# ranok92/gym-ballenv

Measured on AMD Instinct MI355X. Metric: env-steps/sec (whole node), batch=65536 envs, window=10; achieved HBM GB/s, higher is better.
Workload: dtype int16x2+f64

## Files before the change

gym-ballenv_amd/csrc/ballenv.hip:

```cpp
#include <type_traits>
#include <hip/hip_runtime.h>

#include <math.h>
#include <algorithm>
#include <mutex>
#include <new>
#include <stdint.h>
#include <stdio.h>
#include <stdlib.h>
#include <string.h>

#include "ballenv.h"
#include "internal.h"
#include "philox.h"
#include "policy_core.h"

namespace {

constexpr uint32_t PURPOSE_STEP_OBS = 1, PURPOSE_ACTION = 2, PURPOSE_RESET = 3, PURPOSE_SAMPLE = 4;
constexpr int REJECT_LIMIT = 4096;
constexpr int CS = 16;
constexpr int CD = 8;
constexpr int HW_MAX = 63;

enum Mode { MODE_STEP = 0, MODE_RESET = 1, MODE_OBSERVE = 2 };

struct Tables {
  int32_t goal[BE_MAX_GOALS];
  int32_t action[BE_MAX_ACTIONS];
  int32_t speed[BE_MAX_DYNAMIC];
  int32_t strip_obs_x, strip_obs_y, strip_goal_x, strip_goal_y, strip_agent_x, strip_agent_y;
  int32_t radius_obstacle, radius_agent;
  uint8_t n_other[BE_MAX_GOALS];
  uint8_t other[BE_MAX_GOALS][BE_MAX_GOALS];
  uint8_t hw[HW_MAX + 1];
};

constexpr int SPAN_N = 72;
struct TablesX {
  Tables t;
  uint64_t span[SPAN_N];
};
static_assert(sizeof(Tables) % 16 == 0 && sizeof(TablesX) % 16 == 0, "16-byte table staging");
__host__ __device__ constexpr bool span_fits(int W, int R) {
  return W >= 2 && R >= 0 && W - 1 + 2 * R <= 63 && 2 * R + 2 * (W - 1) - 1 <= SPAN_N;
}

struct KParams {
  int32_t* agent; int32_t* goal; double* prev_dist; double* total_dist;
  double* ep_return; int32_t* ep_len; uint32_t* episode; int32_t* static_obs;
  int32_t* dyn_obs; uint8_t* dyn_goal; uint8_t* obs; float* obs_f32;
  double* reward; uint8_t* done; const uint8_t* actions; const Tables* tables;
  int32_t n, window, ns, nd, R, speed_x, speed_y, screen_w;
  int32_t screen_h, goal_change, certainty, time_limit, num_actions, autoreset, gid0, dbg;
  double threshold_goal, time_penalty, static_penalty, dynamic_penalty, min_spawn_dist;
  double inv_g1;
  unsigned long long seed;
  int* status;
  const int16_t* deltas; const int16_t* tape; const uint8_t* mask; const int16_t* reset_tape;
  uint8_t* truncated; uint8_t* terminal_obs; double* final_return; int32_t* final_len;
  double* stats;
  int32_t reset_tape_len;
  int32_t min_spawn_d2;
  uint32_t amx, amy;
  int32_t num_goals;
  int32_t prev_read;
  int32_t steps;
  int32_t pol_bytes, pol_actions;
  const uint8_t* pol_img;
  const uint8_t* obs_in;
  uint8_t* obs_last;
  uint8_t* act_out; float* logp_out; float* value_out;
  unsigned long long pol_seed;
  uint32_t* pool;
};

constexpr uint32_t POOL_VALID = 1u, POOL_REJ = 2u;
constexpr int PB_ROWS = 0, PB_AGENT = 3, PB_GOAL = 4, PB_PREV = 6, PB_TOTAL = 8, PB_OBS = 10;
__host__ __device__ constexpr int pool_body_words(int ns, int nd) { return (PB_OBS + ns + nd + 3) & ~3; }
__host__ __device__ constexpr int64_t pool_bytes_per_env(int ns, int nd) { return 2 * (8 + 4ll * pool_body_words(ns, nd)); }
static_assert(pool_body_words(13, 5) == 28, "the fixed-shape kernels' 112-byte entry body");
__device__ __forceinline__ uint32_t pool_body(uint32_t n, uint32_t x, int nbw) { return 16u * n + x * (4u * (uint32_t)nbw); }
template <class T>
__device__ __forceinline__ T pool_ld(const uint32_t* pool, uint32_t off, uint32_t imm = 0) {
  return *reinterpret_cast<const T*>(reinterpret_cast<const char*>(pool) + (size_t)off + imm);
}
template <class T>
__device__ __forceinline__ void pool_st(uint32_t* pool, uint32_t off, T v, uint32_t imm = 0) {
  *reinterpret_cast<T*>(reinterpret_cast<char*>(pool) + (size_t)off + imm) = v;
}
#ifndef BE_POOL_MODE
#define BE_POOL_MODE 1
#endif
__device__ __forceinline__ uint32_t u4w(const uint4& v, int k) { return k == 0 ? v.x : k == 1 ? v.y : k == 2 ? v.z : v.w; }
__device__ __forceinline__ double u2d(uint32_t lo, uint32_t hi) {
  return __longlong_as_double((long long)(((unsigned long long)hi << 32) | lo));
}
constexpr int64_t POOL_MAX_ENVS = 1ll << 22;

#define BE_DIAG_UNIT_STEP 1
#include "diag.h"

__device__ __forceinline__ int px(int32_t p) { return (int)(int16_t)(p & 0xFFFF); }
__device__ __forceinline__ int py(int32_t p) { return p >> 16; }
__device__ __forceinline__ int32_t pk(int x, int y) {
  return (int32_t)(((uint32_t)x & 0xFFFFu) | ((uint32_t)y << 16));
}
__device__ __forceinline__ uint32_t d2u(int dx, int dy) {
  uint32_t ax = (uint32_t)abs(dx), ay = (uint32_t)abs(dy);
  return ax * ax + ay * ay;
}
__device__ __forceinline__ int d2i(int dx, int dy) { return dx * dx + dy * dy; }
template <class T>
__device__ __forceinline__ T ld_s(const T* base, uint32_t idx) {
  return *reinterpret_cast<const T*>(reinterpret_cast<const char*>(base) + (size_t)(idx * (uint32_t)sizeof(T)));
}
#ifndef BE_S2_CT
#define BE_S2_CT 256
#endif
constexpr int S2_CT = BE_S2_CT;
constexpr int ST_PLAIN = 0, ST_WT = 1;
template <class T>
__device__ __forceinline__ void st_wt(T* p, T v) {
  __hip_atomic_store(p, v, __ATOMIC_RELAXED, __HIP_MEMORY_SCOPE_AGENT);
}
template <class T>
__device__ __forceinline__ T& ld_s_ptr(T* base, uint32_t idx) {
  return *reinterpret_cast<T*>(reinterpret_cast<char*>(base) + (size_t)(idx * (uint32_t)sizeof(T)));
}
template <class T>
__device__ __forceinline__ void st_ws(T* base, uint32_t idx, T v) {
  st_wt(&ld_s_ptr(base, idx), v);
}
__device__ __forceinline__ int isqrt_small(int n) {
  int s = (int)__builtin_amdgcn_sqrtf((float)n);
  if (s * s > n) --s;
  if ((s + 1) * (s + 1) <= n) ++s;
  return s;
}
__device__ __forceinline__ int floordiv(int a, int b) { return a >= 0 ? a / b : -((-a + b - 1) / b); }

typedef short v2s __attribute__((ext_vector_type(2)));

__device__ __forceinline__ uint32_t pick_word(const u4& b, int w) {
  return w == 0 ? b.x : (w == 1 ? b.y : (w == 2 ? b.z : b.w));
}
__device__ __forceinline__ uint32_t pick_field(const u4& b, int j) {
  constexpr uint32_t M = 0xFFFFFFu;
  return j == 0 ? (b.x & M)
       : j == 1 ? (__builtin_amdgcn_alignbit(b.y, b.x, 24) & M)
       : j == 2 ? (__builtin_amdgcn_alignbit(b.z, b.y, 16) & M)
       : j == 3 ? (b.z >> 8) : (b.w & M);
}
__device__ __forceinline__ int map_range(uint32_t r, int lo, int hi) {
  return lo + (int)__umulhi(r, (uint32_t)(hi - lo));
}

struct ResetDraws {
  const int16_t* tape; int32_t len; int32_t n; int32_t env; int32_t cursor;
  uint32_t gid; uint32_t episode; unsigned long long seed;
  int* status;
  __device__ int draw(int lo, int hi) {
    int k = cursor++;
    if (tape) {
      if (k >= len) { atomicOr(status, BE_STATUS_RESET_TAPE_EXHAUSTED); return lo; }
      return tape[(int64_t)k * n + env];
    }
    u4 b = philox(gid, episode, 0u, tag(PURPOSE_RESET, (uint32_t)k >> 2), seed);
    return map_range(pick_word(b, k & 3), lo, hi);
  }
};

__device__ __forceinline__ double sqrt_int(double x) {
  const double y = __builtin_amdgcn_rsq(x);
  double g = x * y, h = y * 0.5;
  const double r = __builtin_fma(-h, g, 0.5);
  g = __builtin_fma(g, r, g);
  h = __builtin_fma(h, r, h);
  double d = __builtin_fma(-g, g, x);
  g = __builtin_fma(d, h, g);
  d = __builtin_fma(-g, g, x);
  g = __builtin_fma(d, h, g);
  return x == 0.0 ? x : g;
}

__device__ __forceinline__ double calc_dist(int x1, int y1, int x2, int y2) {
  double dx = (double)(x1 - x2), dy = (double)(y1 - y2);
  return sqrt_int(dx * dx + dy * dy);
}
__device__ __forceinline__ double calc_dist_lib(int x1, int y1, int x2, int y2) {
  double dx = (double)(x1 - x2), dy = (double)(y1 - y2);
  return sqrt(dx * dx + dy * dy);
}

struct Win {
  int x0, y0;
  int sx, sy;
  int w;
  int kr;
  int R, R2;
  __device__ Win(const KParams& p, int ax, int ay) {
    w = p.window; const int h = w / 2;
    sx = p.speed_x; sy = p.speed_y;
    x0 = ax - sx * h; y0 = ay - sy * h;
    kr = w > 1 ? w - 1 : 1;
    R = p.R; R2 = R * R;
  }
  __device__ __forceinline__ bool near(int ox, int oy, int& f, int& e) const {
    f = ox - x0; e = oy - y0;
    const int cx = min(max(f, 0), sx * (w - 1));
    const int cy = min(max(e, 0), sy * (kr - 1));
    return d2u(f - cx, e - cy) <= (uint32_t)R2;
  }
};

__device__ __forceinline__ int quadrant(int ax, int ay, int gx, int gy) {
  const int dx = gx - ax, dy = gy - ay;
  if (dx >= 0 && dy >= 0) return 1;
  if (dx < 0 && dy >= 0) return 0;
  if (dx < 0 && dy < 0) return 3;
  return 2;
}

__device__ __forceinline__ uint32_t lds_bytes(const void* lo, const void* hi) {
  return (uint32_t)(uintptr_t)hi - (uint32_t)(uintptr_t)lo;
}

template <int BLOCK>
struct NearList {
  uint32_t* base; int cnt;
  __device__ __forceinline__ void push(int f, int e) {
    base[cnt * BLOCK] = (uint32_t)(f & 0xFFFF) | ((uint32_t)e << 16);
    ++cnt;
  }
  __device__ __forceinline__ void push_if(bool c, int f, int e) {
    if (c) push(f, e);
  }
  __device__ __forceinline__ void get(int n, int& f, int& e) const {
    const uint32_t v = base[n * BLOCK];
    f = (int)(int16_t)(v & 0xFFFF); e = (int)v >> 16;
  }
};

template <int WT> struct Geo {
  static constexpr int K = WT > 1 ? WT - 1 : 1;
  static constexpr int NW = (WT * WT + 31) / 32 + 1;
  static constexpr int F = 4 + WT * WT;
};

template <int WT, int BLOCK, bool HWT = false>
__device__ __forceinline__ void raster_rows(const NearList<BLOCK>& nl, const Win& g, uint32_t (&rows)[Geo<WT>::K],
                                            const uint8_t* hwt = nullptr) {
  constexpr int K = Geo<WT>::K;
#pragma unroll
  for (int k = 0; k < K; ++k) rows[k] = 0u;
  if constexpr (HWT) {
    for (int n = 0; n < nl.cnt; ++n) {
      int f, e;
      nl.get(n, f, e);
      f += WT / 2; e += WT / 2;
#pragma unroll
      for (int k = 0; k < K; ++k) {
        const int ady = abs(e - k);
        const int hw = hwt[min(ady, HW_MAX)];
        const int lo = max(f - hw, 0), hi = min(f + hw, WT - 1);
        rows[k] |= (ady <= g.R && lo <= hi) ? (2u << hi) - (1u << lo) : 0u;
      }
    }
    return;
// ... 1141 lines not shown
        const int nr = min(RCAP, nres - r0);
        if (r0 > 0) {
          if (valid && lead && s_slot_of[el] >= r0 && s_slot_of[el] < r0 + RCAP) {
            const int s = s_slot_of[el] - r0;
            s_reset_el[s] = (int16_t)el; s_reset_ep[s] = episode + 1u;
          }
          __syncthreads();
        }
        if (tid < nr) {
          const int e_l = s_reset_el[tid];
          const int ir = blk0 + e_l;
          const uint32_t ep = s_reset_ep[tid];
          const uint32_t g_id = (uint32_t)p.gid0 + (uint32_t)ir;
          const int W = p.screen_w, H = p.screen_h;
          const u4 b0 = philox(g_id, ep, 0u, tag(PURPOSE_RESET, 0), p.seed);
          const int rgx = map_range(b0.x, W - t.strip_goal_x, W), rgy = map_range(b0.y, H - t.strip_goal_y, H);
          int rax = map_range(b0.z, 0, t.strip_agent_x), ray = map_range(b0.w, 0, t.strip_agent_y);
          const double dist = calc_dist(rgx, rgy, rax, ray);
          for (int r = 0; calc_dist(rgx, rgy, rax, ray) < p.min_spawn_dist; ++r) {
            if (r >= REJECT_LIMIT - 1) { atomicOr(p.status, BE_STATUS_REJECTION_LIMIT); break; }
            const u4 b = philox(g_id, ep, 0u, tag(PURPOSE_RESET, 1 + r), p.seed);
            rax = map_range(b.x, 0, t.strip_agent_x); ray = map_range(b.y, 0, t.strip_agent_y);
          }
          p.agent[ir] = pk(rax, ray);
          p.goal[ir] = pk(rgx, rgy);
          p.prev_dist[ir] = dist;
          p.total_dist[ir] = calc_dist(rax, ray, rgx, rgy);
          p.ep_return[ir] = 0.0;
          p.ep_len[ir] = 0;
          p.episode[ir] = ep;
          s_reset_agent[tid] = pk(rax, ray);
          s_reset_goal[tid] = pk(rgx, rgy);
#pragma unroll
          for (int k = 0; k < KR; ++k) s_rows[tid][k] = 0u;
        }
        __syncthreads();
        DIAG(12);
        const int per = Ns + Nd;
        const int R = t.radius_obstacle + t.radius_agent;
        const int rx = R, ry2 = t.radius_obstacle + 2 * t.radius_agent;
        for (int it = tid; it < nr * per; it += BLOCK_THREADS) {
          const int s = it / per, k = it - s * per;
          const int ir = blk0 + s_reset_el[s];
          const uint32_t ep = s_reset_ep[s];
          const uint32_t g_id = (uint32_t)p.gid0 + (uint32_t)ir;
          const int rax = px(s_reset_agent[s]), ray = py(s_reset_agent[s]);
          const int rgx = px(s_reset_goal[s]), rgy = py(s_reset_goal[s]);
          const int W = p.screen_w, H = p.screen_h;
          int ox, oy;
          if (k < Ns) {
            for (int at = 0;; ++at) {
              const u4 b = philox(g_id, ep, 0u, tag(PURPOSE_RESET, (1u << 22) | ((uint32_t)k << 12) | (uint32_t)at), p.seed);
              ox = map_range(b.x, t.strip_obs_x, W - t.strip_obs_x);
              oy = map_range(b.y, t.strip_obs_y, H - t.strip_obs_y);
              const bool ra = abs(ox - rax) < rx && 2 * abs(oy - ray) < ry2;
              const bool rg = abs(ox - rgx) < rx && 2 * abs(oy - rgy) < ry2;
              if (!ra && !rg) break;
              if (at >= REJECT_LIMIT - 1) { atomicOr(p.status, BE_STATUS_REJECTION_LIMIT); break; }
            }
            (p.static_obs + (size_t)k * N)[ir] = pk(ox, oy);
          } else {
            const int kd = k - Ns;
            const u4 b = philox(g_id, ep, 0u, tag(PURPOSE_RESET, (2u << 22) | ((uint32_t)kd << 12)), p.seed);
            ox = map_range(b.x, t.strip_obs_x, W - t.strip_obs_x);
            oy = map_range(b.y, t.strip_obs_y, H - t.strip_obs_y);
            (p.dyn_obs + (size_t)kd * N)[ir] = pk(ox, oy);
            (p.dyn_goal + (size_t)kd * N)[ir] = (uint8_t)kd;
          }
          const Win g(p, rax, ray);
          int f, e;
          if (g.near(ox, oy, f, e)) raster_one_lds<WT>(s_rows[s], g, f, e);
        }
        __syncthreads();
        DIAG(13);
        if (tid < nr) {
          uint32_t rows[Geo<WT>::K], fl[Geo<WT>::NW];
#pragma unroll
          for (int k = 0; k < Geo<WT>::K; ++k) rows[k] = s_rows[tid][k];
          flatten<WT>(rows, fl);
          const int e_l = s_reset_el[tid];
          const int32_t ag = s_reset_agent[tid], go = s_reset_goal[tid];
          stage_full_row<WT>(stage + e_l * F, fl, quadrant(px(ag), py(ag), px(go), py(go)));
        }
        __syncthreads();
        DIAG(14);
      }
    }
    DIAG(5);
    const int nvalid = min(EPB, N - blk0);
    copy_out<BLOCK_THREADS>(stage, F, nvalid, (int64_t)blk0, p.obs, p.obs_f32);
  } else {
    if (valid && lead) {
      const int F = 4 + p.window * p.window;
      const Win g(p, ax, ay);
      write_row_generic<BLOCK_THREADS>(nl, g, quadrant(ax, ay, gx, gy), p.obs ? p.obs + (int64_t)i * F : nullptr,
                                       p.obs_f32 ? p.obs_f32 + (int64_t)i * F : nullptr);
    }
    if (MODE == MODE_STEP && (tid & 63) == 0) s_ws[tid >> 6] = ws;
    __syncthreads();
  }

  DIAG(6);
  if (MODE == MODE_STEP && p.stats && tid == 0) {
    WaveStats b = s_ws[0];
#pragma unroll
    for (int w = 1; w < BLOCK_THREADS / 64; ++w) {
      const WaveStats& o = s_ws[w];
      b.n += o.n; b.s1 += o.s1; b.s2 += o.s2; b.sl += o.sl; b.mn = fmin(b.mn, o.mn); b.mx = fmax(b.mx, o.mx);
    }
    if (b.n > 0.0) {
      double* slot = p.stats + (size_t)blockIdx.x * 8;
      slot[0] += b.n; slot[1] += b.s1; slot[2] += b.s2; slot[3] += b.sl;
      slot[4] = fmin(slot[4], b.mn); slot[5] = fmax(slot[5], b.mx);
    }
  }
}

__device__ __forceinline__ uint32_t mul24_byte(uint32_t x, uint32_t k, int sel) {
  uint32_t r;
  switch (sel) {
    case 0: asm("v_mul_u32_u24_sdwa %0, %1, %2 dst_sel:DWORD dst_unused:UNUSED_PAD src0_sel:BYTE_0 src1_sel:DWORD" : "=v"(r) : "v"(x), "v"(k)); break;
    case 1: asm("v_mul_u32_u24_sdwa %0, %1, %2 dst_sel:DWORD dst_unused:UNUSED_PAD src0_sel:BYTE_1 src1_sel:DWORD" : "=v"(r) : "v"(x), "v"(k)); break;
    case 2: asm("v_mul_u32_u24_sdwa %0, %1, %2 dst_sel:DWORD dst_unused:UNUSED_PAD src0_sel:BYTE_2 src1_sel:DWORD" : "=v"(r) : "v"(x), "v"(k)); break;
    default: asm("v_mul_u32_u24_sdwa %0, %1, %2 dst_sel:DWORD dst_unused:UNUSED_PAD src0_sel:BYTE_3 src1_sel:DWORD" : "=v"(r) : "v"(x), "v"(k)); break;
  }
  return r;
}
__device__ __forceinline__ uint32_t pair_or(uint32_t x) {
  return x | (uint32_t)__builtin_amdgcn_update_dpp(0, (int)x, 0xB1, 0xF, 0xF, false);
}

template <int WT, int NSC, int NDC, bool POOL = false>
__global__ __launch_bounds__(S2_CT, 2) void step2_kernel(KParams p) {
  constexpr int CT = S2_CT;
  constexpr int L = 2, EPW = 64 / L, EPB = CT / L, NWAVE = CT / 64;
  constexpr int SS = (NSC + L - 1) / L, SD = (NDC + L - 1) / L;
  constexpr int KR = Geo<WT>::K, F = Geo<WT>::F, NW = Geo<WT>::NW;
  constexpr int NQ = F / 8, HQ = (NQ + 1) / 2;
  static_assert(WT == 10 && F == 104 && NW == 5, "the half-row word split below is laid out for W = 10");
  static_assert(NDC <= 5, "one Philox block of 24-bit fields");
  static_assert(16 * KR >= (64 / (NSC + NDC)) * (KR + 4), "wave reset scratch");
  extern __shared__ __align__(16) uint8_t smem[];
  __shared__ __align__(16) TablesX t_wave[NWAVE];
  __shared__ uint32_t s_rows[NWAVE][16 * KR];
  constexpr int TW = (int)(sizeof(TablesX) / 16);

  DIAG(0);
  if (DBG(DBG_EXIT_ENTRY)) return;
  const int N = p.n, tid = (int)threadIdx.x, w = tid >> 6, lane = tid & 63, h = lane & 1;
  const int blk0 = (int)blockIdx.x * EPB, i = blk0 + (tid >> 1), e0 = blk0 + w * EPW;
  uint8_t* stage_blk = smem + (size_t)(SS + SD + 1) * CT * 4;
  const bool valid = i < N;
  const uint32_t ic = (uint32_t)min(i, N - 1), gid = (uint32_t)p.gid0 + (uint32_t)i;
  NearList<CT> nl{reinterpret_cast<uint32_t*>(smem) + tid, 0};
  Tables& t = t_wave[w].t;
  const uint64_t* span = t_wave[w].span;
  uint8_t* stage = stage_blk + (size_t)w * EPW * F;
  constexpr int TB = 64;
  const int tt0 = lane;

  constexpr int TL = (TW + TB - 1) / TB;
  uint4 tword[TL];
#pragma unroll
  for (int j = 0; j < TL; ++j)
    tword[j] = ld_s(reinterpret_cast<const uint4*>(p.tables), (uint32_t)min(tt0 + j * TB, TW - 1));
  const uint32_t episode = ld_s(p.episode, ic);
  const int len0 = ld_s(p.ep_len, ic);
  const int32_t agent0 = ld_s(p.agent, ic), goal0 = ld_s(p.goal, ic);
  int32_t dp[SD], so[SS];
  int dgi[SD];
#pragma unroll
  for (int j = 0; j < SD; ++j) {
    const uint32_t e = (uint32_t)min(L * j + h, NDC - 1) * (uint32_t)N + ic;
    dp[j] = ld_s(p.dyn_obs, e);
    dgi[j] = ld_s(p.dyn_goal, e);
  }
#pragma unroll
  for (int j = 0; j < SS; ++j) so[j] = ld_s(p.static_obs, (uint32_t)min(L * j + h, NSC - 1) * (uint32_t)N + ic);
  const double old_dist = p.prev_read ? ld_s(p.prev_dist, ic) : calc_dist(px(goal0), py(goal0), px(agent0), py(agent0));
  const double total = ld_s(p.total_dist, ic);
  double ret = ld_s(p.ep_return, ic);
  const int a = ld_s(p.actions, ic);
  double* const slot = p.stats ? p.stats + (size_t)(e0 / 32) * 8 : nullptr;
  double2 sp0 = make_double2(0.0, 0.0), sp1 = sp0, sp2 = sp0;
  if (slot && lane == 0 && e0 < N) {
    sp0 = reinterpret_cast<const double2*>(slot)[0];
    sp1 = reinterpret_cast<const double2*>(slot)[1];
    sp2 = reinterpret_cast<const double2*>(slot)[2];
  }
#pragma unroll
  for (int j = 0; j < TL; ++j) reinterpret_cast<uint4*>(&t_wave[w])[min(tt0 + j * TB, TW - 1)] = tword[j];
  __builtin_amdgcn_fence(__ATOMIC_RELEASE, "wavefront");
  __builtin_amdgcn_wave_barrier();
  __builtin_amdgcn_fence(__ATOMIC_ACQUIRE, "wavefront");
  DIAG(1);
  if (DBG(DBG_EXIT_BARRIER)) return;
  if (DBG(DBG_WAIT_LOADS)) {
    __builtin_amdgcn_s_waitcnt(0);
    DIAG(15);
  }

  int counter = (int)((double)len0 * p.inv_g1);
  counter = len0 - counter * (p.goal_change + 1);
  if (counter < 0) counter += p.goal_change + 1;
  if (counter > p.goal_change) counter -= p.goal_change + 1;
  const bool change = counter >= p.goal_change;
  const u4 b0 = DBG(DBG_NO_PHILOX) ? u4{gid, episode, (uint32_t)len0, gid ^ episode}
                                   : philox(gid, episode, (uint32_t)len0, tag(PURPOSE_STEP_OBS, 0u), p.seed);
  DIAG(7);
  uint32_t st_flags = 0u;
  int ngs[SD];
  int32_t dnew[SD];
#pragma unroll
  for (int j = 0; j < SD; ++j) {
    const int k = L * j + h;
    const bool real = k < NDC;
    int ox = px(dp[j]), oy = py(dp[j]);
    const uint32_t f = h ? pick_field(b0, min(L * j + 1, 4)) : pick_field(b0, L * j);
    uint32_t fl = 0u;
    ngs[j] = dyn_move_fixed(p, t, ox, oy, dgi[j], t.speed[min(k, NDC - 1)], change, f, fl);
    st_flags |= real ? fl : 0u;
    dnew[j] = pk(ox, oy);
  }
  DIAG(11);
  st_flags |= a >= p.num_actions ? (uint32_t)BE_STATUS_BAD_ACTION : 0u;
  const uint32_t sh = 2u * (uint32_t)(a < p.num_actions ? a : 0);
  int ax = min(max(px(agent0) + (int)((p.amx >> sh) & 3u) - 1, 0), p.screen_w);
  int ay = min(max(py(agent0) + (int)((p.amy >> sh) & 3u) - 1, 0), p.screen_h);
  int gx = px(goal0), gy = py(goal0);
  const Win g0(p, 0, 0);
  const uint32_t R2 = (uint32_t)g0.R2;
  const NearBox nb0(g0);
  typedef unsigned short v2u __attribute__((ext_vector_type(2)));
  const v2s boxo = {(short)(WT / 2 + g0.R), (short)(WT / 2 + g0.R)};
  const v2u boxw = {(unsigned short)nb0.bw, (unsigned short)nb0.bh};
  const v2s agv = __builtin_bit_cast(v2s, pk(ax, ay));
  const double dist = calc_dist(gx, gy, ax, ay);
  const double rbase = (0.0 - p.time_penalty) + (old_dist - dist) / total;
  DIAG(8);
  bool hs = false, hd = false;
  uint32_t* nlp = nl.base;
  auto obstacle_pk = [&](int32_t opk, bool real, bool& hit) {
    const v2s d = __builtin_elementwise_sub_sat(__builtin_bit_cast(v2s, opk), agv);
    hit |= real & ((uint32_t)dot2_sq(d) <= R2);
    const v2u b = __builtin_bit_cast(v2u, __builtin_elementwise_add_sat(d, boxo));
    const v2u over = __builtin_elementwise_sub_sat(b, boxw);
    *nlp = __builtin_bit_cast(uint32_t, d);
    const uint32_t in = __builtin_elementwise_sub_sat(1u, __builtin_bit_cast(uint32_t, over) | (real ? 0u : 1u));
    nlp += CT * in;
  };
#pragma unroll
  for (int j = 0; j < SD; ++j) obstacle_pk(dnew[j], L * j + h < NDC, hd);
#pragma unroll
  for (int j = 0; j < SS; ++j) obstacle_pk(so[j], L * j + h < NSC, hs);
  nl.cnt = (int)(lds_bytes(nl.base, nlp) / (CT * 4u));
  hs = pair_or((uint32_t)hs) != 0u;
  hd = pair_or((uint32_t)hd) != 0u;
  DIAG(10);

  double reward = rbase;
  if (hs) reward -= p.static_penalty;
  else if (hd) reward -= p.dynamic_penalty;
  ret += reward;
  const int len = len0 + 1;
  const bool env_done = (dist < p.threshold_goal) || hs || hd;
  const bool trunc = p.time_limit > 0 && len >= p.time_limit;
  const bool done = env_done || trunc;
  const bool do_reset = valid && done && p.autoreset;
  const bool ptry = POOL && do_reset && p.pool != nullptr;
  uint2 q_tv = make_uint2(0u, 0u);
  uint4 qb[7];
#if BE_POOL_MODE == 1 || BE_POOL_MODE == 6
  if constexpr (POOL)
#if BE_POOL_MODE == 6
  if (__ballot(ptry))
#endif
  if (ptry) {
    const uint32_t x = ((episode + 1u) & 1u) * (uint32_t)N + (uint32_t)i;
    q_tv = pool_ld<uint2>(p.pool, x * 8u);
    const uint32_t bo = pool_body((uint32_t)N, x, 28);
#pragma unroll
    for (int j = 0; j < 7; ++j) qb[j] = pool_ld<uint4>(p.pool, bo, 16u * j);
    __builtin_amdgcn_s_waitcnt(0);
  }
#ifdef BE_DIAG_STAMPS
  if (__ballot(ptry)) DIAG(9);
#endif
#endif
  if (valid) {
    const uint32_t iu = (uint32_t)i;
    st_ws(p.reward, iu, reward);
    st_ws(p.ep_return, iu, ret);
    st_ws(p.agent, iu, pk(ax, ay));
    st_ws(p.ep_len, iu, len);
    if (p.done) st_ws(p.done, iu, (uint8_t)done);
    if (p.truncated) st_ws(p.truncated, iu, (uint8_t)(trunc && !env_done));
    st_ws(p.prev_dist, iu, dist);
    if (done) {
      if (p.final_return) st_ws(p.final_return, iu, ret);
      if (p.final_len) st_ws(p.final_len, iu, len);
    }
#pragma unroll
    for (int j = 0; j < SD; ++j) {
      const int k = L * j + h;
      if (k < NDC) {
        st_wt(&ld_s_ptr(p.dyn_obs, (uint32_t)k * (uint32_t)N + (uint32_t)i), dnew[j]);
        if (change) st_wt(&ld_s_ptr(p.dyn_goal, (uint32_t)k * (uint32_t)N + (uint32_t)i), (uint8_t)ngs[j]);
      }
    }
  }
  DIAG(2);
  if (__ballot(st_flags != 0u)) {
    uint32_t f = st_flags;
#pragma unroll
    for (int o = 32; o > 0; o >>= 1) f |= (uint32_t)__shfl_xor((int)f, o);
    if (lane == 0) atomicOr(p.status, (int)f);
  }
  if (DBG(DBG_EXIT_PHYSICS)) return;

  uint32_t xrows[KR];
#pragma unroll
  for (int k = 0; k < KR; ++k) xrows[k] = 0u;
  if (do_reset && p.terminal_obs) {
    uint32_t rows[KR], flat[NW];
    raster_rows_span<WT, CT>(nl, p.R, rows, span);
#pragma unroll
    for (int k = 0; k < KR; ++k) rows[k] = pair_or(rows[k]);
    flatten<WT>(rows, flat);
    if (!h) write_row_global<WT>(p.terminal_obs + (int64_t)i * F, flat, quadrant(ax, ay, gx, gy));
  }
  bool hit = false;
#if BE_POOL_MODE == 5
  const unsigned long long m0 = DBG(DBG_NO_RESET) ? 0ull : __ballot(do_reset && h == 0);
  if (m0) {
  if (POOL) {
    if (ptry) {
      const uint32_t x = ((episode + 1u) & 1u) * (uint32_t)N + (uint32_t)i;
      q_tv = pool_ld<uint2>(p.pool, x * 8u);
      const uint32_t bo = pool_body((uint32_t)N, x, 28);
#pragma unroll
      for (int j = 0; j < 7; ++j) qb[j] = pool_ld<uint4>(p.pool, bo, 16u * j);
    }
#else
  if (__ballot(ptry)) {
#endif
    hit = ptry && q_tv.x == episode + 1u && (q_tv.y & POOL_VALID) != 0u;
    if (hit) {
      auto qw = [&](int k) -> uint32_t { return u4w(qb[k >> 2], k & 3); };
      const uint32_t iu = (uint32_t)i;
      const int32_t ag = (int32_t)qw(PB_AGENT), go = (int32_t)qw(PB_GOAL);
      st_ws(p.ep_return, iu, 0.0);
      st_ws(p.ep_len, iu, 0);
      st_ws(p.agent, iu, ag);
      st_ws(p.prev_dist, iu, u2d(qw(PB_PREV), qw(PB_PREV + 1)));
      st_ws(p.goal, iu, go);
      st_ws(p.total_dist, iu, u2d(qw(PB_TOTAL), qw(PB_TOTAL + 1)));
      st_ws(p.episode, iu, episode + 1u);
#pragma unroll
      for (int j = 0; j < SD; ++j) {
        const int k = L * j + h;
        const uint32_t o = h ? qw(PB_OBS + NSC + min(L * j + 1, NDC - 1)) : qw(PB_OBS + NSC + L * j);
        if (k < NDC) {
          st_ws(p.dyn_obs, (uint32_t)k * (uint32_t)N + iu, (int32_t)o);
          st_ws(p.dyn_goal, (uint32_t)k * (uint32_t)N + iu, (uint8_t)k);
        }
      }
#pragma unroll
      for (int j = 0; j < SS; ++j) {
        const int k = L * j + h;
        const uint32_t o = h ? qw(PB_OBS + min(L * j + 1, NSC - 1)) : qw(PB_OBS + L * j);
        if (k < NSC) st_ws(p.static_obs, (uint32_t)k * (uint32_t)N + iu, (int32_t)o);
      }
      ax = px(ag); ay = py(ag); gx = px(go); gy = py(go);
#pragma unroll
      for (int k = 0; k < KR; ++k) xrows[k] = (qw(PB_ROWS + k / 3) >> (10 * (k % 3))) & 0x3FFu;
      nl.cnt = 0;
    }
    if (__ballot(hit && (q_tv.y & POOL_REJ)) && lane == 0) atomicOr(p.status, BE_STATUS_REJECTION_LIMIT);
  }
  const unsigned long long m = DBG(DBG_NO_RESET) ? 0ull : __ballot(do_reset && !hit && h == 0);
  if (m) {
    auto osink = [&](int, int k, int il, int32_t o) {
      if (k < NSC) {
        st_ws(p.static_obs, (uint32_t)k * (uint32_t)N + (uint32_t)il, o);
      } else {
        st_ws(p.dyn_obs, (uint32_t)(k - NSC) * (uint32_t)N + (uint32_t)il, o);
        st_ws(p.dyn_goal, (uint32_t)(k - NSC) * (uint32_t)N + (uint32_t)il, (uint8_t)(k - NSC));
      }
    };
    auto esink = [&](int, int32_t ag, int32_t go, int32_t a0) {
      double prev;
      const double td = reset_dists(ag, go, a0, prev);
      const uint32_t iu = (uint32_t)i;
      st_ws(p.ep_return, iu, 0.0);
      st_ws(p.ep_len, iu, 0);
      st_ws(p.agent, iu, ag);
      st_ws(p.prev_dist, iu, prev);
      st_ws(p.goal, iu, go);
      st_ws(p.total_dist, iu, td);
      st_ws(p.episode, iu, episode + 1u);
    };
    if (!(m & (m - 1)))
      wave_resets<WT, NSC, NDC, 1, decltype(osink)&, decltype(esink)&, L>(p, t, m, i, gid, episode, ax, ay, gx, gy,
                                                                        nl.cnt, xrows, &s_rows[w][0], osink, esink, span);
    else
      wave_resets<WT, NSC, NDC, 64, decltype(osink)&, decltype(esink)&, L>(p, t, m, i, gid, episode, ax, ay, gx, gy,
                                                                         nl.cnt, xrows, &s_rows[w][0], osink, esink, span);
  }
#if BE_POOL_MODE == 5
  }
#endif
  DIAG(3);
  if (DBG(DBG_NO_OBS)) return;
  if (DBG(DBG_NO_RASTER)) nl.cnt = 0;

  {
    uint32_t rows[KR];
    raster_rows_span<WT, CT>(nl, p.R, rows, span, xrows);
    const uint32_t P0 = pair_or(rows[0] | (rows[1] << 10) | (rows[2] << 20));
    const uint32_t P1 = pair_or(rows[3] | (rows[4] << 10) | (rows[5] << 20));
    const uint32_t P2 = pair_or(rows[6] | (rows[7] << 10) | (rows[8] << 20));
    const uint32_t vlo = h ? ((P1 >> 6) & 0xFFFFF0u) | (P2 << 24) : ((P0 << 4) & 0x3FF0u) | (P0 << 14);
    const uint32_t vhi = h ? P2 >> 8 : (P0 >> 18) | (P1 << 12);
    const unsigned long long c = (((unsigned long long)vhi << 32) | vlo) >> (6 * h);
    const uint32_t clo = (uint32_t)c, chi = (uint32_t)(c >> 32);
    const uint32_t ne0 = clo & 0x0F0F0F0Fu, no0 = (clo >> 4) & 0x0F0F0F0Fu;
    const uint32_t ne1 = chi & 0x0F0F0F0Fu, no1 = (chi >> 4) & 0x0F0F0F0Fu;
    const uint32_t kx = 0x00204081u;
    auto word = [&](int jj) -> uint32_t {
      const int b = jj >> 1;
      const uint32_t src = (jj & 1) ? (b < 4 ? no0 : no1) : (b < 4 ? ne0 : ne1);
      return mul24_byte(src, kx, b & 3) & 0x01010101u;
    };
    const uint32_t sx = (uint32_t)(gx - ax) >> 31, sy = (uint32_t)(gy - ay) >> 31;
    const uint32_t onehot = 1u << ((sy << 4) | ((sx ^ sy ^ 1u) << 3));
    uint2* dst = reinterpret_cast<uint2*>(stage + (tid & 62) / 2 * F) + HQ * h;
#pragma unroll
    for (int q = 0; q < HQ; ++q) {
      const uint32_t w0 = q == 0 ? (h ? word(0) : onehot) : word(2 * q);
      if (q < NQ - HQ || !h) dst[q] = make_uint2(w0, word(2 * q + 1));
    }
  }
  DIAG(4);
  __builtin_amdgcn_fence(__ATOMIC_RELEASE, "wavefront");
  __builtin_amdgcn_wave_barrier();
  __builtin_amdgcn_fence(__ATOMIC_ACQUIRE, "wavefront");
  DIAG(5);
  if (!DBG(DBG_NO_COPY)) {
    const int e0u = __builtin_amdgcn_readfirstlane(e0);
    if (e0u + EPW <= N && p.obs && !p.obs_f32)
      copy_wave_full<EPW * F / 16>(stage, p.obs + (size_t)e0u * F, lane);
    else
      copy_out<64>(stage, F, max(0, min(EPW, N - e0u)), (int64_t)e0u, p.obs, p.obs_f32, lane);
  }
  WaveStats ws{0.0, 0.0, 0.0, 0.0, INFINITY, -INFINITY};
  if (slot && !DBG(DBG_NO_STATS)) ws = wave_stats(done && valid && h == 0, ret, len);
  if (slot && lane == 0 && ws.n > 0.0) {
    reinterpret_cast<double2*>(slot)[0] = make_double2(sp0.x + ws.n, sp0.y + ws.s1);
    reinterpret_cast<double2*>(slot)[1] = make_double2(sp1.x + ws.s2, sp1.y + ws.sl);
    reinterpret_cast<double2*>(slot)[2] = make_double2(fmin(sp2.x, ws.mn), fmax(sp2.y, ws.mx));
  }
  DIAG(6);
}

template <int L>
__device__ __forceinline__ uint32_t lane_group_or(uint32_t x) {
  static_assert(L == 4 || L == 8, "L must be 4 or 8");
  x |= (uint32_t)__builtin_amdgcn_update_dpp(0, (int)x, 0xB1, 0xF, 0xF, false);
  x |= (uint32_t)__builtin_amdgcn_update_dpp(0, (int)x, 0x4E, 0xF, 0xF, false);
  if constexpr (L == 8) x |= (uint32_t)__builtin_amdgcn_update_dpp(0, (int)x, 0x141, 0xF, 0xF, false);
  return x;
}

template <int WT, int NSC, int NDC, int L, bool POOL = false>
__global__ __launch_bounds__(32 * L) void stepw_kernel(KParams p) {
  constexpr int CT = 32 * L, EPW = 64 / L, NWAVE = CT / 64;
  constexpr int SS = (NSC + L - 1) / L, SD = (NDC + L - 1) / L;
  constexpr int KR = Geo<WT>::K, F = Geo<WT>::F;
  constexpr int BPL = (F + L - 1) / L;
  constexpr int WB = EPW * F, SW = (WB + 15) & ~15;
  static_assert(WT * KR <= 20, "packed rows: 20 bits + the two collision flags");
  static_assert(NDC <= 5, "one Philox block of 24-bit fields");
  static_assert(16 * KR >= (64 / (NSC + NDC)) * (KR + 4), "wave reset scratch");
  static_assert(WB % 8 == 0, "a wave's rows are whole 8-byte words");
  __shared__ Tables t_wave[NWAVE];
  __shared__ uint32_t s_rows[NWAVE][16 * KR];
  __shared__ __align__(16) uint8_t s_stage[NWAVE][SW];
  __shared__ double s_fret[32];
  __shared__ int32_t s_flen[32];
  __shared__ uint8_t s_fin[32];
  constexpr int TW = (int)(sizeof(Tables) / 4);

  if (DBG(DBG_EXIT_ENTRY)) return;
  PH_INIT;
  const int N = p.n, tid = (int)threadIdx.x, w = tid >> 6, lane = tid & 63, h = lane & (L - 1);
  const int el = tid / L, blk0 = (int)blockIdx.x * 32, i = blk0 + el, e0 = blk0 + w * EPW;
  const bool valid = i < N;
  const uint32_t ic = (uint32_t)min(i, N - 1), gid = (uint32_t)p.gid0 + (uint32_t)i;
  uint8_t* stage = &s_stage[w][0];
  Tables& t = t_wave[w];

  constexpr int TL = (TW + 63) / 64;
  uint32_t tword[TL];
#pragma unroll
  for (int j = 0; j < TL; ++j)
    tword[j] = ld_s(reinterpret_cast<const uint32_t*>(p.tables), (uint32_t)min(lane + j * 64, TW - 1));
  const uint32_t episode = ld_s(p.episode, ic);
  const int len0 = ld_s(p.ep_len, ic);
  const int32_t agent0 = ld_s(p.agent, ic), goal0 = ld_s(p.goal, ic);
  int32_t dp[SD], so[SS];
  int dgi[SD];
#pragma unroll
  for (int j = 0; j < SD; ++j) {
    uint32_t kn = (uint32_t)min(L * j + h, NDC - 1) * (uint32_t)N;
    asm volatile("" : "+v"(kn));
    const uint32_t e = kn + ic;
    dp[j] = ld_s(p.dyn_obs, e);
    dgi[j] = ld_s(p.dyn_goal, e);
  }
#pragma unroll
  for (int j = 0; j < SS; ++j) {
    uint32_t kn = (uint32_t)min(L * j + h, NSC - 1) * (uint32_t)N;
    asm volatile("" : "+v"(kn));
    so[j] = ld_s(p.static_obs, kn + ic);
  }
  const double old_read = ld_s(p.prev_dist, ic);
  const double total = ld_s(p.total_dist, ic);
  double ret = ld_s(p.ep_return, ic);
  const int a = ld_s(p.actions, ic);
  __builtin_amdgcn_sched_barrier(0);
  const double old_dist = p.prev_read ? old_read : calc_dist(px(goal0), py(goal0), px(agent0), py(agent0));
  double* const slot = p.stats ? p.stats + (size_t)blockIdx.x * 8 : nullptr;
  double2 sp0 = make_double2(0.0, 0.0), sp1 = sp0, sp2 = sp0;
  if (slot && tid == 0) {
    sp0 = reinterpret_cast<const double2*>(slot)[0];
    sp1 = reinterpret_cast<const double2*>(slot)[1];
    sp2 = reinterpret_cast<const double2*>(slot)[2];
  }
#pragma unroll
  for (int j = 0; j < TL; ++j) reinterpret_cast<uint32_t*>(&t)[min(lane + j * 64, TW - 1)] = tword[j];
  __builtin_amdgcn_fence(__ATOMIC_RELEASE, "wavefront");
  __builtin_amdgcn_wave_barrier();
  __builtin_amdgcn_fence(__ATOMIC_ACQUIRE, "wavefront");
  if (DBG(DBG_EXIT_BARRIER)) {
    if (valid && (agent0 ^ goal0 ^ so[0] ^ dp[0] ^ len0 ^ a ^ (int)old_dist ^ (int)ret) == 0x7fffffff) p.obs[i] = 1;
    return;
  }
  if (DBG(DBG_WAIT_LOADS)) __builtin_amdgcn_s_waitcnt(0);
  PH(0);

  int counter = (int)((double)len0 * p.inv_g1);
  counter = len0 - counter * (p.goal_change + 1);
  if (counter < 0) counter += p.goal_change + 1;
  if (counter > p.goal_change) counter -= p.goal_change + 1;
  const bool change = counter >= p.goal_change;
  const u4 b0 = DBG(DBG_NO_PHILOX) ? u4{gid, episode, 7u, 9u} : philox(gid, episode, (uint32_t)len0, tag(PURPOSE_STEP_OBS, 0u), p.seed);
  uint32_t st_flags = 0u;
  int ngs[SD];
  int32_t dnew[SD];
#pragma unroll
  for (int j = 0; j < SD; ++j) {
    const int k = L * j + h;
    int ox = px(dp[j]), oy = py(dp[j]);
    uint32_t fl = 0u;
    ngs[j] = dyn_move_fixed(p, t, ox, oy, dgi[j], t.speed[min(k, NDC - 1)], change, pick_field(b0, min(k, 4)), fl);
    st_flags |= k < NDC ? fl : 0u;
    dnew[j] = pk(ox, oy);
  }
  PH(1);
  st_flags |= a >= p.num_actions ? (uint32_t)BE_STATUS_BAD_ACTION : 0u;
  const uint32_t sh = 2u * (uint32_t)(a < p.num_actions ? a : 0);
  int ax = min(max(px(agent0) + (int)((p.amx >> sh) & 3u) - 1, 0), p.screen_w);
  int ay = min(max(py(agent0) + (int)((p.amy >> sh) & 3u) - 1, 0), p.screen_h);
  int gx = px(goal0), gy = py(goal0);
  const int R = p.R;
  const uint32_t R2 = (uint32_t)(R * R);
  const v2s agv = __builtin_bit_cast(v2s, pk(ax, ay));
  const double dist = calc_dist(gx, gy, ax, ay);
  const double rbase = (0.0 - p.time_penalty) + (old_dist - dist) / total;
  PH(2);

  uint32_t word = 0u;
  auto obstacle = [&](int32_t opk, bool real, uint32_t hit_bit) {
    const v2s d = __builtin_elementwise_sub_sat(__builtin_bit_cast(v2s, opk), agv);
    word |= (real & ((uint32_t)__builtin_amdgcn_sdot2(d, d, 0, false) <= R2)) ? hit_bit : 0u;
    const int f = d.x + WT / 2, e = d.y + WT / 2;
    if (real & ((uint32_t)(f + R) <= (uint32_t)(WT - 1 + 2 * R)) & ((uint32_t)(e + R) <= (uint32_t)(KR - 1 + 2 * R))) {
#pragma unroll
      for (int k = 0; k < KR; ++k) {
        const int ady = abs(e - k);
        const int hw = t.hw[min(ady, HW_MAX)];
        const int lo = max(f - hw, 0), hi = min(f + hw, WT - 1);
        word |= (ady <= R && lo <= hi) ? ((2u << hi) - (1u << lo)) << (WT * k) : 0u;
      }
    }
  };
#pragma unroll
  for (int j = 0; j < SD; ++j) obstacle(dnew[j], L * j + h < NDC, 1u << 21);
#pragma unroll
  for (int j = 0; j < SS; ++j) obstacle(so[j], L * j + h < NSC, 1u << 20);
  word = lane_group_or<L>(word);
  const bool hs = (word >> 20) & 1u, hd = (word >> 21) & 1u;
  uint32_t rows = word & 0xFFFFFu;
  PH(3);

  double reward = rbase;
  if (hs) reward -= p.static_penalty;
  else if (hd) reward -= p.dynamic_penalty;
  ret += reward;
  const int len = len0 + 1;
  const bool env_done = (dist < p.threshold_goal) || hs || hd;
  const bool trunc = p.time_limit > 0 && len >= p.time_limit;
  const bool done = env_done || trunc;
  const bool do_reset = valid && done && p.autoreset;
  const bool ptry = POOL && do_reset && p.pool != nullptr;
// ... 1738 lines not shown
```

Baseline: 11.39 billion.

## Split step tail into fast no-done path and wave-uniform reset path

Restructures the kernel tail into a lambda instantiated twice. Waves with no done env take a lean path that skips pool loads, terminal-obs and reset logic and the stats fold. Waves with any done env issue pool loads unconditionally and early, overlapping them with rasterization, and reuse one raster for both terminal and regular observations. The cost is larger code and extra pool loads for lanes that do not reset.

```diff
diff --git a/gym-ballenv_amd/csrc/ballenv.hip b/gym-ballenv_amd/csrc/ballenv.hip
--- a/gym-ballenv_amd/csrc/ballenv.hip
+++ b/gym-ballenv_amd/csrc/ballenv.hip
@@ -115,6 +115,12 @@
 __device__ __forceinline__ T ld_s(const T* base, uint32_t idx) {
   return *reinterpret_cast<const T*>(reinterpret_cast<const char*>(base) + (size_t)(idx * (uint32_t)sizeof(T)));
 }
+#ifndef BE_S2_FIN_LOAD
+#define BE_S2_FIN_LOAD 1
+#endif
+#ifndef BE_S2_FIN_ORDER
+#define BE_S2_FIN_ORDER 3
+#endif
 #ifndef BE_S2_CT
 #define BE_S2_CT 256
 #endif
@@ -1562,6 +1568,11 @@
   uint8_t* stage_blk = smem + (size_t)(SS + SD + 1) * CT * 4;
   const bool valid = i < N;
   const uint32_t ic = (uint32_t)min(i, N - 1), gid = (uint32_t)p.gid0 + (uint32_t)i;
+  const struct {
+    double *reward, *ep_return, *prev_dist; int32_t *agent, *ep_len, *dyn_obs;
+    uint8_t *dyn_goal, *done, *truncated, *obs; float* obs_f32; int* status; const uint32_t* pool;
+  } ptr = {p.reward, p.ep_return, p.prev_dist, p.agent, p.ep_len, p.dyn_obs,
+         p.dyn_goal, p.done, p.truncated, p.obs, p.obs_f32, p.status, p.pool};
   NearList<CT> nl{reinterpret_cast<uint32_t*>(smem) + tid, 0};
   Tables& t = t_wave[w].t;
   const uint64_t* span = t_wave[w].span;
@@ -1677,156 +1688,7 @@
   const bool trunc = p.time_limit > 0 && len >= p.time_limit;
   const bool done = env_done || trunc;
   const bool do_reset = valid && done && p.autoreset;
-  const bool ptry = POOL && do_reset && p.pool != nullptr;
-  uint2 q_tv = make_uint2(0u, 0u);
-  uint4 qb[7];
-#if BE_POOL_MODE == 1 || BE_POOL_MODE == 6
-  if constexpr (POOL)
-#if BE_POOL_MODE == 6
-  if (__ballot(ptry))
-#endif
-  if (ptry) {
-    const uint32_t x = ((episode + 1u) & 1u) * (uint32_t)N + (uint32_t)i;
-    q_tv = pool_ld<uint2>(p.pool, x * 8u);
-    const uint32_t bo = pool_body((uint32_t)N, x, 28);
-#pragma unroll
-    for (int j = 0; j < 7; ++j) qb[j] = pool_ld<uint4>(p.pool, bo, 16u * j);
-    __builtin_amdgcn_s_waitcnt(0);
-  }
-#ifdef BE_DIAG_STAMPS
-  if (__ballot(ptry)) DIAG(9);
-#endif
-#endif
-  if (valid) {
-    const uint32_t iu = (uint32_t)i;
-    st_ws(p.reward, iu, reward);
-    st_ws(p.ep_return, iu, ret);
-    st_ws(p.agent, iu, pk(ax, ay));
-    st_ws(p.ep_len, iu, len);
-    if (p.done) st_ws(p.done, iu, (uint8_t)done);
-    if (p.truncated) st_ws(p.truncated, iu, (uint8_t)(trunc && !env_done));
-    st_ws(p.prev_dist, iu, dist);
-    if (done) {
-      if (p.final_return) st_ws(p.final_return, iu, ret);
-      if (p.final_len) st_ws(p.final_len, iu, len);
-    }
-#pragma unroll
-    for (int j = 0; j < SD; ++j) {
-      const int k = L * j + h;
-      if (k < NDC) {
-        st_wt(&ld_s_ptr(p.dyn_obs, (uint32_t)k * (uint32_t)N + (uint32_t)i), dnew[j]);
-        if (change) st_wt(&ld_s_ptr(p.dyn_goal, (uint32_t)k * (uint32_t)N + (uint32_t)i), (uint8_t)ngs[j]);
-      }
-    }
-  }
-  DIAG(2);
-  if (__ballot(st_flags != 0u)) {
-    uint32_t f = st_flags;
-#pragma unroll
-    for (int o = 32; o > 0; o >>= 1) f |= (uint32_t)__shfl_xor((int)f, o);
-    if (lane == 0) atomicOr(p.status, (int)f);
-  }
-  if (DBG(DBG_EXIT_PHYSICS)) return;
-
-  uint32_t xrows[KR];
-#pragma unroll
-  for (int k = 0; k < KR; ++k) xrows[k] = 0u;
-  if (do_reset && p.terminal_obs) {
-    uint32_t rows[KR], flat[NW];
-    raster_rows_span<WT, CT>(nl, p.R, rows, span);
-#pragma unroll
-    for (int k = 0; k < KR; ++k) rows[k] = pair_or(rows[k]);
-    flatten<WT>(rows, flat);
-    if (!h) write_row_global<WT>(p.terminal_obs + (int64_t)i * F, flat, quadrant(ax, ay, gx, gy));
-  }
-  bool hit = false;
-#if BE_POOL_MODE == 5
-  const unsigned long long m0 = DBG(DBG_NO_RESET) ? 0ull : __ballot(do_reset && h == 0);
-  if (m0) {
-  if (POOL) {
-    if (ptry) {
-      const uint32_t x = ((episode + 1u) & 1u) * (uint32_t)N + (uint32_t)i;
-      q_tv = pool_ld<uint2>(p.pool, x * 8u);
-      const uint32_t bo = pool_body((uint32_t)N, x, 28);
-#pragma unroll
-      for (int j = 0; j < 7; ++j) qb[j] = pool_ld<uint4>(p.pool, bo, 16u * j);
-    }
-#else
-  if (__ballot(ptry)) {
-#endif
-    hit = ptry && q_tv.x == episode + 1u && (q_tv.y & POOL_VALID) != 0u;
-    if (hit) {
-      auto qw = [&](int k) -> uint32_t { return u4w(qb[k >> 2], k & 3); };
-      const uint32_t iu = (uint32_t)i;
-      const int32_t ag = (int32_t)qw(PB_AGENT), go = (int32_t)qw(PB_GOAL);
-      st_ws(p.ep_return, iu, 0.0);
-      st_ws(p.ep_len, iu, 0);
-      st_ws(p.agent, iu, ag);
-      st_ws(p.prev_dist, iu, u2d(qw(PB_PREV), qw(PB_PREV + 1)));
-      st_ws(p.goal, iu, go);
-      st_ws(p.total_dist, iu, u2d(qw(PB_TOTAL), qw(PB_TOTAL + 1)));
-      st_ws(p.episode, iu, episode + 1u);
-#pragma unroll
-      for (int j = 0; j < SD; ++j) {
-        const int k = L * j + h;
-        const uint32_t o = h ? qw(PB_OBS + NSC + min(L * j + 1, NDC - 1)) : qw(PB_OBS + NSC + L * j);
-        if (k < NDC) {
-          st_ws(p.dyn_obs, (uint32_t)k * (uint32_t)N + iu, (int32_t)o);
-          st_ws(p.dyn_goal, (uint32_t)k * (uint32_t)N + iu, (uint8_t)k);
-        }
-      }
-#pragma unroll
-      for (int j = 0; j < SS; ++j) {
-        const int k = L * j + h;
-        const uint32_t o = h ? qw(PB_OBS + min(L * j + 1, NSC - 1)) : qw(PB_OBS + L * j);
-        if (k < NSC) st_ws(p.static_obs, (uint32_t)k * (uint32_t)N + iu, (int32_t)o);
-      }
-      ax = px(ag); ay = py(ag); gx = px(go); gy = py(go);
-#pragma unroll
-      for (int k = 0; k < KR; ++k) xrows[k] = (qw(PB_ROWS + k / 3) >> (10 * (k % 3))) & 0x3FFu;
-      nl.cnt = 0;
-    }
-    if (__ballot(hit && (q_tv.y & POOL_REJ)) && lane == 0) atomicOr(p.status, BE_STATUS_REJECTION_LIMIT);
-  }
-  const unsigned long long m = DBG(DBG_NO_RESET) ? 0ull : __ballot(do_reset && !hit && h == 0);
-  if (m) {
-    auto osink = [&](int, int k, int il, int32_t o) {
-      if (k < NSC) {
-        st_ws(p.static_obs, (uint32_t)k * (uint32_t)N + (uint32_t)il, o);
-      } else {
-        st_ws(p.dyn_obs, (uint32_t)(k - NSC) * (uint32_t)N + (uint32_t)il, o);
-        st_ws(p.dyn_goal, (uint32_t)(k - NSC) * (uint32_t)N + (uint32_t)il, (uint8_t)(k - NSC));
-      }
-    };
-    auto esink = [&](int, int32_t ag, int32_t go, int32_t a0) {
-      double prev;
-      const double td = reset_dists(ag, go, a0, prev);
-      const uint32_t iu = (uint32_t)i;
-      st_ws(p.ep_return, iu, 0.0);
-      st_ws(p.ep_len, iu, 0);
-      st_ws(p.agent, iu, ag);
-      st_ws(p.prev_dist, iu, prev);
-      st_ws(p.goal, iu, go);
-      st_ws(p.total_dist, iu, td);
-      st_ws(p.episode, iu, episode + 1u);
-    };
-    if (!(m & (m - 1)))
-      wave_resets<WT, NSC, NDC, 1, decltype(osink)&, decltype(esink)&, L>(p, t, m, i, gid, episode, ax, ay, gx, gy,
-                                                                        nl.cnt, xrows, &s_rows[w][0], osink, esink, span);
-    else
-      wave_resets<WT, NSC, NDC, 64, decltype(osink)&, decltype(esink)&, L>(p, t, m, i, gid, episode, ax, ay, gx, gy,
-                                                                         nl.cnt, xrows, &s_rows[w][0], osink, esink, span);
-  }
-#if BE_POOL_MODE == 5
-  }
-#endif
-  DIAG(3);
-  if (DBG(DBG_NO_OBS)) return;
-  if (DBG(DBG_NO_RASTER)) nl.cnt = 0;
-
-  {
-    uint32_t rows[KR];
-    raster_rows_span<WT, CT>(nl, p.R, rows, span, xrows);
+  auto obs_out = [&](const uint32_t (&rows)[KR]) __attribute__((always_inline)) {
     const uint32_t P0 = pair_or(rows[0] | (rows[1] << 10) | (rows[2] << 20));
     const uint32_t P1 = pair_or(rows[3] | (rows[4] << 10) | (rows[5] << 20));
     const uint32_t P2 = pair_or(rows[6] | (rows[7] << 10) | (rows[8] << 20));
@@ -1850,27 +1712,196 @@
       const uint32_t w0 = q == 0 ? (h ? word(0) : onehot) : word(2 * q);
       if (q < NQ - HQ || !h) dst[q] = make_uint2(w0, word(2 * q + 1));
     }
-  }
-  DIAG(4);
-  __builtin_amdgcn_fence(__ATOMIC_RELEASE, "wavefront");
-  __builtin_amdgcn_wave_barrier();
-  __builtin_amdgcn_fence(__ATOMIC_ACQUIRE, "wavefront");
-  DIAG(5);
-  if (!DBG(DBG_NO_COPY)) {
-    const int e0u = __builtin_amdgcn_readfirstlane(e0);
-    if (e0u + EPW <= N && p.obs && !p.obs_f32)
-      copy_wave_full<EPW * F / 16>(stage, p.obs + (size_t)e0u * F, lane);
-    else
-      copy_out<64>(stage, F, max(0, min(EPW, N - e0u)), (int64_t)e0u, p.obs, p.obs_f32, lane);
-  }
-  WaveStats ws{0.0, 0.0, 0.0, 0.0, INFINITY, -INFINITY};
-  if (slot && !DBG(DBG_NO_STATS)) ws = wave_stats(done && valid && h == 0, ret, len);
-  if (slot && lane == 0 && ws.n > 0.0) {
-    reinterpret_cast<double2*>(slot)[0] = make_double2(sp0.x + ws.n, sp0.y + ws.s1);
-    reinterpret_cast<double2*>(slot)[1] = make_double2(sp1.x + ws.s2, sp1.y + ws.sl);
-    reinterpret_cast<double2*>(slot)[2] = make_double2(fmin(sp2.x, ws.mn), fmax(sp2.y, ws.mx));
-  }
-  DIAG(6);
+    DIAG(4);
+    __builtin_amdgcn_fence(__ATOMIC_RELEASE, "wavefront");
+    __builtin_amdgcn_wave_barrier();
+    __builtin_amdgcn_fence(__ATOMIC_ACQUIRE, "wavefront");
+    DIAG(5);
+    if (!DBG(DBG_NO_COPY)) {
+      const int e0u = __builtin_amdgcn_readfirstlane(e0);
+      if (e0u + EPW <= N && ptr.obs && !ptr.obs_f32)
+        copy_wave_full<EPW * F / 16>(stage, ptr.obs + (size_t)e0u * F, lane);
+      else
+        copy_out<64>(stage, F, max(0, min(EPW, N - e0u)), (int64_t)e0u, ptr.obs, ptr.obs_f32, lane);
+    }
+  };
+  auto tail = [&](auto fin_c) __attribute__((always_inline)) {
+    constexpr bool FIN = decltype(fin_c)::value;
+    uint2 q_tv = make_uint2(0u, 0u);
+    uint4 qb[7];
+    if constexpr (FIN && POOL) {
+#if BE_S2_FIN_LOAD == 1
+      const uint32_t x = ((episode + 1u) & 1u) * (uint32_t)N + ic;
+      q_tv = pool_ld<uint2>(ptr.pool, x * 8u);
+      const uint32_t bo = pool_body((uint32_t)N, x, 28);
+#pragma unroll
+      for (int j = 0; j < 7; ++j) qb[j] = pool_ld<uint4>(ptr.pool, bo, 16u * j);
+#else
+      if (do_reset) {
+        const uint32_t x = ((episode + 1u) & 1u) * (uint32_t)N + (uint32_t)i;
+        q_tv = pool_ld<uint2>(ptr.pool, x * 8u);
+        const uint32_t bo = pool_body((uint32_t)N, x, 28);
+#pragma unroll
+        for (int j = 0; j < 7; ++j) qb[j] = pool_ld<uint4>(ptr.pool, bo, 16u * j);
+        __builtin_amdgcn_s_waitcnt(0);
+      }
+#endif
+    }
+    if (valid) {
+      const uint32_t iu = (uint32_t)i;
+      st_ws(ptr.reward, iu, reward);
+      st_ws(ptr.ep_return, iu, ret);
+      st_ws(ptr.agent, iu, pk(ax, ay));
+      st_ws(ptr.ep_len, iu, len);
+      if (ptr.done) st_ws(ptr.done, iu, (uint8_t)(FIN && done));
+      if (ptr.truncated) st_ws(ptr.truncated, iu, (uint8_t)(FIN && trunc && !env_done));
+      st_ws(ptr.prev_dist, iu, dist);
+      if constexpr (FIN) {
+        if (done) {
+          if (p.final_return) st_ws(p.final_return, iu, ret);
+          if (p.final_len) st_ws(p.final_len, iu, len);
+        }
+      }
+#pragma unroll
+      for (int j = 0; j < SD; ++j) {
+        const int k = L * j + h;
+        if (k < NDC) {
+          st_wt(&ld_s_ptr(ptr.dyn_obs, (uint32_t)k * (uint32_t)N + (uint32_t)i), dnew[j]);
+          if (change) st_wt(&ld_s_ptr(ptr.dyn_goal, (uint32_t)k * (uint32_t)N + (uint32_t)i), (uint8_t)ngs[j]);
+        }
+      }
+    }
+    DIAG(2);
+    if (__ballot(st_flags != 0u)) {
+      uint32_t f = st_flags;
+#pragma unroll
+      for (int o = 32; o > 0; o >>= 1) f |= (uint32_t)__shfl_xor((int)f, o);
+      if (lane == 0) atomicOr(ptr.status, (int)f);
+    }
+    if (DBG(DBG_EXIT_PHYSICS)) return;
+
+    if constexpr (!FIN) {
+      DIAG(3);
+      if (DBG(DBG_NO_OBS)) return;
+      if (DBG(DBG_NO_RASTER)) nl.cnt = 0;
+      uint32_t rows[KR];
+      raster_rows_span<WT, CT>(nl, p.R, rows, span);
+      obs_out(rows);
+      DIAG(6);
+      return;
+    } else {
+      auto fold = [&]() __attribute__((always_inline)) {
+        if (slot && !DBG(DBG_NO_STATS)) {
+          const WaveStats ws = wave_stats(done && valid && h == 0, ret, len);
+          if (lane == 0 && ws.n > 0.0) {
+            reinterpret_cast<double2*>(slot)[0] = make_double2(sp0.x + ws.n, sp0.y + ws.s1);
+            reinterpret_cast<double2*>(slot)[1] = make_double2(sp1.x + ws.s2, sp1.y + ws.sl);
+            reinterpret_cast<double2*>(slot)[2] = make_double2(fmin(sp2.x, ws.mn), fmax(sp2.y, ws.mx));
+          }
+        }
+      };
+#if BE_S2_FIN_ORDER == 1
+      fold();
+#endif
+      if (DBG(DBG_NO_RASTER)) nl.cnt = 0;
+      uint32_t xrows[KR];
+      raster_rows_span<WT, CT>(nl, p.R, xrows, span);
+      const bool tobs = do_reset && p.terminal_obs != nullptr;
+      uint32_t tflat[NW];
+      const int tquad = quadrant(ax, ay, gx, gy);
+      if (p.terminal_obs) {
+        uint32_t rows[KR];
+#pragma unroll
+        for (int k = 0; k < KR; ++k) rows[k] = pair_or(xrows[k]);
+        flatten<WT>(rows, tflat);
+      }
+#if BE_S2_FIN_ORDER == 2
+      fold();
+#endif
+      bool hit = false;
+      if constexpr (POOL) {
+#if BE_S2_FIN_LOAD == 1
+        asm volatile("" :: "v"(q_tv.x), "v"(q_tv.y));
+#pragma unroll
+        for (int j = 0; j < 7; ++j) asm volatile("" :: "v"(qb[j].x), "v"(qb[j].y), "v"(qb[j].z), "v"(qb[j].w));
+#endif
+        hit = do_reset && q_tv.x == episode + 1u && (q_tv.y & POOL_VALID) != 0u;
+#ifdef BE_DIAG_STAMPS
+        if (__ballot(do_reset)) DIAG(9);
+#endif
+        if (hit) {
+          auto qw = [&](int k) -> uint32_t { return u4w(qb[k >> 2], k & 3); };
+          const uint32_t iu = (uint32_t)i;
+          const int32_t ag = (int32_t)qw(PB_AGENT), go = (int32_t)qw(PB_GOAL);
+          st_ws(ptr.ep_return, iu, 0.0);
+          st_ws(ptr.ep_len, iu, 0);
+          st_ws(ptr.agent, iu, ag);
+          st_ws(ptr.prev_dist, iu, u2d(qw(PB_PREV), qw(PB_PREV + 1)));
+          st_ws(p.goal, iu, go);
+          st_ws(p.total_dist, iu, u2d(qw(PB_TOTAL), qw(PB_TOTAL + 1)));
+          st_ws(p.episode, iu, episode + 1u);
+#pragma unroll
+          for (int j = 0; j < SD; ++j) {
+            const int k = L * j + h;
+            const uint32_t o = h ? qw(PB_OBS + NSC + min(L * j + 1, NDC - 1)) : qw(PB_OBS + NSC + L * j);
+            if (k < NDC) {
+              st_ws(ptr.dyn_obs, (uint32_t)k * (uint32_t)N + iu, (int32_t)o);
+              st_ws(ptr.dyn_goal, (uint32_t)k * (uint32_t)N + iu, (uint8_t)k);
+            }
+          }
+#pragma unroll
+          for (int j = 0; j < SS; ++j) {
+            const int k = L * j + h;
+            const uint32_t o = h ? qw(PB_OBS + min(L * j + 1, NSC - 1)) : qw(PB_OBS + L * j);
+            if (k < NSC) st_ws(p.static_obs, (uint32_t)k * (uint32_t)N + iu, (int32_t)o);
+          }
+          ax = px(ag); ay = py(ag); gx = px(go); gy = py(go);
+#pragma unroll
+          for (int k = 0; k < KR; ++k) xrows[k] = (qw(PB_ROWS + k / 3) >> (10 * (k % 3))) & 0x3FFu;
+        }
+        if (__ballot(hit && (q_tv.y & POOL_REJ)) && lane == 0) atomicOr(ptr.status, BE_STATUS_REJECTION_LIMIT);
+      }
+      if (tobs && !h) write_row_global<WT>(p.terminal_obs + (int64_t)i * F, tflat, tquad);
+      const unsigned long long m = DBG(DBG_NO_RESET) ? 0ull : __ballot(do_reset && !hit && h == 0);
+      if (m) {
+        auto osink = [&](int, int k, int il, int32_t o) {
+          if (k < NSC) {
+            st_ws(p.static_obs, (uint32_t)k * (uint32_t)N + (uint32_t)il, o);
+          } else {
+            st_ws(ptr.dyn_obs, (uint32_t)(k - NSC) * (uint32_t)N + (uint32_t)il, o);
+            st_ws(ptr.dyn_goal, (uint32_t)(k - NSC) * (uint32_t)N + (uint32_t)il, (uint8_t)(k - NSC));
+          }
+        };
+        auto esink = [&](int, int32_t ag, int32_t go, int32_t a0) {
+          double prev;
+          const double td = reset_dists(ag, go, a0, prev);
+          const uint32_t iu = (uint32_t)i;
+          st_ws(ptr.ep_return, iu, 0.0);
+          st_ws(ptr.ep_len, iu, 0);
+          st_ws(ptr.agent, iu, ag);
+          st_ws(ptr.prev_dist, iu, prev);
+          st_ws(p.goal, iu, go);
+          st_ws(p.total_dist, iu, td);
+          st_ws(p.episode, iu, episode + 1u);
+        };
+        if (!(m & (m - 1)))
+          wave_resets<WT, NSC, NDC, 1, decltype(osink)&, decltype(esink)&, L>(p, t, m, i, gid, episode, ax, ay, gx, gy,
+                                                                            nl.cnt, xrows, &s_rows[w][0], osink, esink, span);
+        else
+          wave_resets<WT, NSC, NDC, 64, decltype(osink)&, decltype(esink)&, L>(p, t, m, i, gid, episode, ax, ay, gx, gy,
+                                                                             nl.cnt, xrows, &s_rows[w][0], osink, esink, span);
+      }
+      DIAG(3);
+      if (DBG(DBG_NO_OBS)) return;
+      obs_out(xrows);
+#if BE_S2_FIN_ORDER == 3
+      fold();
+#endif
+      DIAG(6);
+    }
+  };
+  if (__ballot(valid && done)) tail(std::true_type{});
+  else tail(std::false_type{});
 }
 
 template <int L>
```

Result: faster. 12.06 billion, median of 6 (+5.9%).
